# DavidBluecame/libYafaRay

Hardware: AMD Instinct MI355X
Metric: Mrays/sec + Msamples/sec, 1920×1080×64spp path-trace at 1/2/4/8 GPUs (higher is better)
Workload: dtype f32

## Files before the change

libyafaray_amd/csrc/kernels.hip:

```cpp

#include <hip/hip_runtime.h>
#include <cstdlib>
#include <string>
#include "devmath.h"
#include "photonheap.h"
#include "devscene.h"
#include "texeval.h"

namespace yafamd
{

#ifndef YAF_TRACE_BLOCK
#define YAF_TRACE_BLOCK 128
#endif
#ifndef YAF_SHADE_MIN_WAVES
#define YAF_SHADE_MIN_WAVES 4
#endif
#ifndef YAF_SHADE_LEAN_WAVES
#define YAF_SHADE_LEAN_WAVES 4
#endif
#ifndef YAF_SHADE_PREFETCH
#define YAF_SHADE_PREFETCH 1
#endif
constexpr int kTraceBlock = YAF_TRACE_BLOCK;
#ifdef YAF_EXPERIMENTS
constexpr bool kExperiments = true;
#else
constexpr bool kExperiments = false;
#endif
#if defined(YAF_FUSE) && defined(YAF_EXPERIMENTS)
constexpr bool kShadeFused = true;
#else
constexpr bool kShadeFused = false;
#endif
#ifndef YAF_FUSE_LEAN
#define YAF_FUSE_LEAN 0
#endif
constexpr int kShadeBlock = 256;

enum : uint32_t
{
	ST_CAMERA = 0,
	ST_FIRST = 1,
	ST_BOUNCE = 2,
	ST_NORAY = 3
};
enum : uint32_t
{
	F_MATFLAGS = 0xffffu,
	F_SAMPLED = 1u << 16,
	F_CAUSTIC = 1u << 17,
	F_PEND_V0 = 1u << 18,
	F_PEND_ONE = 1u << 19,
// ... 159 lines not shown
	Q.ray_d[3 * (size_t)i] = __builtin_nanf("");
}

constexpr uint32_t kPmSBits = 20, kPmLBits = 11;
__device__ __forceinline__ bool neePm8(const DevScene &S)
{
	return !S.nee_pm16 && (uint32_t)S.spp < (1u << kPmSBits) && S.n_lights <= (1 << kPmLBits);
}
typedef uint32_t u32x2_t __attribute__((ext_vector_type(2)));
#ifdef YAF_CHECKED
__device__ uint32_t g_nee_pm_err = 0;
#define NEE_PM_GUARD(cond) do { if(!(cond)) atomicCAS(&g_nee_pm_err, 0u, (uint32_t)__LINE__); } while(0)
#else
#define NEE_PM_GUARD(cond) do {} while(0)
#endif
__device__ __forceinline__ void neePmStore(const DevScene &S, uint4 *pm, uint32_t j, uint32_t offset, uint32_t sample_idx, uint32_t mode_l)
{
	if(neePm8(S))
	{
		NEE_PM_GUARD(sample_idx - S.base_offset - S.pass_offset < (uint32_t)S.spp);
		u32x2_t w;
		w.x = offset;
		w.y = (sample_idx - S.base_offset - S.pass_offset) | ((mode_l & 1u) << kPmSBits) | ((mode_l >> 8) << (kPmSBits + 1));
#if YAF_NT_STORE2
		__builtin_nontemporal_store(w, reinterpret_cast<u32x2_t *>(pm) + j);
#else
		reinterpret_cast<u32x2_t *>(pm)[j] = w;
#endif
	}
	else stStore2(&pm[j], make_uint4(offset, sample_idx, mode_l, 0u));
// ... 159 lines not shown
	{
		const uint32_t hstart = S.base_offset + S.pass_offset + offset;
		const float lu = haltonNext(3u, hstart, sc.s + 1), lv = haltonNext(5u, hstart, sc.s + 1);
		float u, v;
		lensUv(c, lu, lv, u, v);
		const V3 li = v3(c.dof_rt[0], c.dof_rt[1], c.dof_rt[2]) * u + v3(c.dof_up[0], c.dof_up[1], c.dof_up[2]) * v;
		from = from + li;
		dir = normalize(dir * c.dof_distance - li);
	}
	const uint64_t gid = ((uint64_t)sc.y * (uint64_t)S.width + (uint64_t)sc.x) * (uint64_t)S.spp + (uint64_t)sc.s;
	const uint32_t gid32 = (uint32_t)gid ^ fnv32((uint32_t)(gid >> 32));
	seed = fnv32(gid32 ^ S.rr_seed ^ (S.pass_offset * 0x9e3779b9u)) + 123u;
}

__global__ void __launch_bounds__(256) k_camera(DevScene S, DevPaths P, DevQueues Q, DevCounters cnt,
                                                 const DevJob *jobs, int n_jobs, uint64_t chunk_base, int n)
{
	const int i = blockIdx.x * blockDim.x + threadIdx.x;
	if((uint32_t)i < S.n_seg)
	{
		const uint32_t groups = (uint32_t)n / 256u, rem = (uint32_t)n % 256u, sg = (uint32_t)i, R = S.n_seg;
		cnt.n_active[sg] = (groups / R) * 256u + (sg < groups % R ? 256u : 0u) + (sg == groups % R ? rem : 0u);
		cnt.n_shadow[sg] = 0;
	}
	if(i >= n) return;
	const uint32_t g = (uint32_t)i / 256u;
	const uint32_t a = (g % S.n_seg) * S.cap_a + (g / S.n_seg) * 256u + (uint32_t)i % 256u;
	const SampleCoord sc = sampleAt(S, jobs, n_jobs, chunk_base + (uint64_t)i);
	V3 from, dir;
	float tmin, tmax;
	uint32_t seed;
	cameraRay(S, sc, from, dir, tmin, tmax, seed);
	storeQRay(Q, a, from, dir);
	if(S.cam.ray_tt) Q.ray_tt[a] = make_float2(tmin, tmax);
	if(!S.tree) reinterpret_cast<uint2 *>(P.pr)[a] = make_uint2((uint32_t)i, ST_CAMERA);
	else
	{
		const int cx = sc.x + S.crop_x0, cy = sc.y + S.crop_y0;
		const uint32_t offset = fnv32((uint32_t)cy * fnv32((uint32_t)cx));
		const uint32_t sample_idx = S.base_offset + S.pass_offset + (uint32_t)sc.s;
		Q.slot[a] = i;
		P.thr[a] = make_float4(0.f, 0.f, 0.f, 0.f);
		P.col[a] = make_float4(0.f, 0.f, 0.f, __uint_as_float(ST_CAMERA));
		P.pcol[a] = make_float4(0.f, 0.f, 0.f, __uint_as_float(0u));
		P.pr[a] = make_uint4(offset, sample_idx, 30903u, seed);
	}
}

#ifndef YAF_TOP_STRIDE
#define YAF_TOP_STRIDE 9
// ... 1978 lines not shown
struct ShadeArgs
{
	DevScene S;
	DevPaths Pc;
	DevPaths Pn;
	DevQueues Q;
	DevQueues Qn;
	DevNeeQueue N;
	DevNeeQueue G;
	DevCounters cnt;
	DevCounters cnt_next;
	float4 *samples;
	const DevJob *jobs;
	int n_jobs;
	uint64_t chunk_base;
};

__device__ __forceinline__ void writeSampleAt(const ShadeArgs &A, const SampleCoord &sc, C3 col, float alpha)
{
	if(alpha > 1.f) alpha = 1.f;
	A.samples[((size_t)sc.y * A.S.width + sc.x) * A.S.spp + sc.s] = f4(col, alpha);
}

__device__ __forceinline__ void writeSample(const ShadeArgs &A, uint32_t sid, C3 col, float alpha)
{
	writeSampleAt(A, sampleAt(A.S, A.jobs, A.n_jobs, A.chunk_base + (uint64_t)sid), col, alpha);
}

__device__ __forceinline__ Surf surfFromPrim(const DevScene &S, V3 p, int prim)
{
	Surf s;
// ... 33 lines not shown
				float f = m.tbias;
				if(m.sd_flags & SD_TBIAS_MULT) f *= (float)level;
				from = sp.p + dir * f;
			}
			S.spawn_o[idx] = f4(from, S.ray_min_dist);
			S.spawn_d[idx] = f4(dir, -1.f - (float)additional_depth);
			S.spawn_pr[idx] = make_uint4(pix.x, pix.y, rng.x ^ (0x9e3779b9u * (uint32_t)(2 * level + k + 1)), rng.y + 1u + (uint32_t)k);
			S.node_w[S.node_base + idx] = f4(k == 0 ? so.rcol : so.tcol, 0.f);
			if(k == 0) child.x = (int)(S.node_base + idx);
			else child.y = (int)(S.node_base + idx);
		}
	}
	S.node_child[node] = child;
}

template<bool SMALL, bool EXT, bool FUSED = false, bool LEAN = false, bool DEFER = false>
__global__ void __launch_bounds__(kShadeBlock, EXT ? 1 : (LEAN ? YAF_SHADE_LEAN_WAVES : YAF_SHADE_MIN_WAVES)) k_shade(ShadeArgs A)
{
	extern __shared__ uint4 shade_smem[];
	DevScene S_ = stageTables<SMALL>(A.S, shade_smem);
	if constexpr(LEAN)
	{
		S_.integrator = INT_PATH;
		S_.path_samples = 1;
		S_.do_ao = 0;
		S_.caus_map = 0;
		S_.show_map = 0;
		S_.gather_on = 0;
		S_.n_photons = 0;
		S_.fg_on = 0;
		S_.tree = 0;
		S_.has_attr = 0;
	}
// ... 11 lines not shown
	out.sh_count = &s_count[2];
	out.sh_base = seg * S.cap_s;
	out.Qn = A.Qn;
	out.idx_in_o = !S.tr_shad;
	const bool is_path = S.integrator == INT_PATH;
	const bool is_photon = S.integrator == INT_PHOTON;
	const bool keep_v0 = S.path_samples > 1 || is_photon || S.caus_map;
	const bool ao_after_caustic = S.caus_map && S.integrator == INT_DIRECT;
	const uint32_t n_paths = (uint32_t)max(1, S.path_samples);
	const int K = S.nee_k;
	const uint32_t stride = blockDim.x;
	const bool compact = !(EXT && S.tree);
	PHASE_DECL
#if YAF_SHADE_PREFETCH
	uint2 pr_n = make_uint2(0u, ST_NORAY);
	if(compact && threadIdx.x < n_a) pr_n = reinterpret_cast<const uint2 *>(Pc.pr)[a0 + threadIdx.x];
#endif
	for(uint32_t base_j = 0; base_j < n_a; base_j += stride)
	{
		const bool live = base_j + threadIdx.x < n_a;
		const uint32_t i = a0 + base_j + threadIdx.x;
#if YAF_SHADE_PREFETCH
		const uint2 pr_cur = pr_n;
		if(compact && base_j + stride + threadIdx.x < n_a) pr_n = reinterpret_cast<const uint2 *>(Pc.pr)[i + stride];
#endif
		uint32_t sid = 0, stage = ST_NORAY, flags = 0;
		uint2 pix = make_uint2(0u, 0u), rng = make_uint2(0u, 0u);
		float w = 0.f;
		float4 thr4 = make_float4(0.f, 0.f, 0.f, 0.f), col4 = thr4, pcol4 = thr4, pwo4 = thr4, pthr4 = thr4, pem4 = thr4;
		float4 v0p4 = thr4, v0wo4 = thr4;
		float4 v0a0 = thr4, v0a1 = thr4;
		SampleCoord sc{0, 0, 0};
		if(live)
		{
			if(compact)
			{
#if YAF_SHADE_PREFETCH
				const uint2 pr = pr_cur;
#else
				const uint2 pr = reinterpret_cast<const uint2 *>(Pc.pr)[i];
#endif
				sid = pr.x;
				stage = pr.y;
				sc = sampleAt(S, A.jobs, A.n_jobs, A.chunk_base + (uint64_t)sid);
				pix = make_uint2(fnv32((uint32_t)(sc.y + S.crop_y0) * fnv32((uint32_t)(sc.x + S.crop_x0))),
				                 S.base_offset + S.pass_offset + (uint32_t)sc.s);
			}
			else
			{
				const uint4 pr = Pc.pr[i];
				rng = make_uint2(pr.z, pr.w);
				sid = (uint32_t)A.Q.slot[i];
				pix = make_uint2(pr.x, pr.y);
				col4 = Pc.col[i];
				stage = __float_as_uint(col4.w);
			}
			if(!compact || (stage & 0xffu) != ST_CAMERA)
			{
				if(S.w_live) thr4 = Pc.thr[i];
				else
				{
					const F3 t = reinterpret_cast<const F3 *>(Pc.thr)[i];
					thr4 = make_float4(t.x, t.y, t.z, 0.f);
				}
				pcol4 = Pc.pcol[i];
				if(keep_v0) { v0p4 = Pc.v0p[i]; v0wo4 = Pc.v0wo[i]; }
				if(ATTR && keep_v0) { v0a0 = Pc.v0attr[2 * (size_t)i]; v0a1 = Pc.v0attr[2 * (size_t)i + 1]; }
			}
			w = thr4.w;
			flags = __float_as_uint(pcol4.w);
			if((stage & 0xffu) == ST_FIRST && !(flags & F_SAMPLED)) pwo4 = Pc.pwo[i];
			if(flags & F_PEND_ONE)
			{
				const F3 t = reinterpret_cast<const F3 *>(Pc.pend_thr)[i];
				pthr4 = make_float4(t.x, t.y, t.z, 0.f);
			}
			if(flags & (F_PEND_EMIT | F_AO_EMIT)) pem4 = Pc.pend_emit[i];
		}
		C3 thr = rgb(thr4), col = rgb(col4), pcol = rgb(pcol4);
		const float alpha = 1.f;
		V3 pwo = xyz(pwo4);
		const uint32_t st = stage & 0xffu;
		uint32_t subpath = (stage >> 8) & 0xfffu;
		int depth = (int)(stage >> 20);
		const uint32_t offset = pix.x, sample_idx = pix.y;
		C3 ao_extra = c3(0.f);
		bool col_ld = !compact, col_dirty = false;
		auto loadCol = [&]() {
			if(!col_ld)
			{
				col = (flags & F_COLS) ? rgb(Pc.csmp[sid]) : c3(0.f);
				col_ld = true;
			}
		};

		PHASE(0);
		const int kb = (int)i * K;
// ... 241 lines not shown
					if(S.caustic_path && (s.sampled & (B_SPECULAR | B_GLOSSY | B_FILTER))) flags |= F_CAUSTIC;
					else flags &= ~F_CAUSTIC;
					ray_o = sp.p;
					ray_d = dir;
					want_ray = true;
					stage = ST_BOUNCE | (subpath << 8) | ((uint32_t)depth << 20);
				}
			}
			else end_sub = true;
		}
		if(live && end_sub && !pending)
		{
			if(is_path && (flags & F_V0_DIFFUSE) && subpath + 1 < n_paths) { start_sub = true; ++subpath; }
			else finalize = true;
		}
		if(live && start_sub)
		{
			Surf s0 = (st == ST_CAMERA) ? sp : surfFromPrim(S, xyz(v0p4), __float_as_int(v0p4.w));
			if(ATTR && st != ST_CAMERA) applyAttr(s0, v0a0, v0a1);
			const V3 wo0 = (st == ST_CAMERA) ? wo : xyz(v0wo4);
			const uint32_t offs = n_paths * sample_idx + offset + subpath;
			BsdfSample s;
			s.s_1 = riVdC(offs);
			s.s_2 = ldsDim(S, 2, offs);
			s.flags = B_DIFFUSE | B_REFLECT | B_TRANSMIT;
			s.pdf = 0.f;
			s.sampled = B_NONE;
			V3 dir = v3(0.f, 0.f, 0.f);
			C3 scol = matSample<EXT>(S.mats[s0.mat], s0, wo0, dir, s, w);
			thr = scol * w;
// ... 55 lines not shown
			else
			{
				storeQNoRay(A.Qn, k);
				if(!FUSED && want_nee) reinterpret_cast<F3 *>(A.Qn.ray_o)[k] = F3{sp.p.x, sp.p.y, sp.p.z};
				stage = ST_NORAY | (subpath << 8) | ((uint32_t)depth << 20);
			}
			if(compact) stStoreU2(reinterpret_cast<uint2 *>(Pn.pr) + k, make_uint2(sid, stage));
			else
			{
				stStore(&Pn.pr[k], make_uint4(pix.x, pix.y, rng.x, rng.y));
				stStore(&Pn.col[k], f4(col, __uint_as_float(stage)));
			}
			if(S.w_live) stStore(&Pn.thr[k], f4(thr, w));
			else stStoreF3(Pn.thr, k, thr);
			stStore(&Pn.pcol[k], f4(pcol, __uint_as_float(flags)));
			if((stage & 0xffu) == ST_FIRST && !(flags & F_SAMPLED)) Pn.pwo[k] = f4(pwo, 0.f);
			if(nee_one) reinterpret_cast<F3 *>(Pn.pend_thr)[k] = F3{pend_thr.r, pend_thr.g, pend_thr.b};
			if(flags & (F_PEND_EMIT | F_AO_EMIT)) Pn.pend_emit[k] = f4(emit_pend, 0.f);
			if(keep_v0) { Pn.v0p[k] = v0p4; Pn.v0wo[k] = v0wo4; }
			if(ATTR && keep_v0) { Pn.v0attr[2 * (size_t)k] = v0a0; Pn.v0attr[2 * (size_t)k + 1] = v0a1; }
		}

		PHASE(4);
		if(FUSED)
		{
			const int e0 = (int)k * K;
			const bool all = live && nee_v0, one = live && nee_one;
			const DevMaterial &m = S.mats[sp.mat];
			float4 *ts = S.tr_shad ? Pn.ts : nullptr;
			if(__any(all))
			{
// ... 3285 lines not shown
using namespace yafamd;

extern "C" {

int yafamd_trace_block() { return kTraceBlock; }

int yafamd_shade_fused() { return kShadeFused ? 1 : 0; }
int yafamd_shade_fused_for(const DevScene *S)
{
	if(S->ext) return 0;
	if(kShadeFused) return 1;
	return (YAF_FUSE_LEAN && S->integrator == INT_PATH && S->path_samples <= 1 && !S->do_ao && !S->caus_map && !S->gather_on && !S->show_map &&
	        S->n_photons == 0 && !S->tree && !S->has_attr && !S->no_lean && !S->tr_shad && !S->has_mesh_light) ? 1 : 0;
}

int yafamd_experiments() { return kExperiments ? 1 : 0; }

#ifndef YAF_DEVICE_BUILD
#define YAF_DEVICE_BUILD "arch=? extra=[?] (built outside csrc/Makefile)"
#endif
const char *yafamd_device_build() { return YAF_DEVICE_BUILD
#ifdef YAF_PHASE_TIMING
	" phase-timing"
#endif
	; }

int yafamd_phase_cycles(unsigned long long *out, int n, int reset)
{
#ifdef YAF_PHASE_TIMING
	unsigned long long h[16];
// ... 37 lines not shown
int yafamd_nee_blocks_per_cu()
{
	int nb = 0;
	if(hipOccupancyMaxActiveBlocksPerMultiprocessor(&nb, (k_nee<true, false>), kShadeBlock, 8192) != hipSuccess) nb = 0;
	return nb;
}

int yafamd_shade_blocks_per_cu()
{
	int nb = 0;
	if(hipOccupancyMaxActiveBlocksPerMultiprocessor(&nb, (k_shade<true, false>), kShadeBlock, 8192) != hipSuccess) nb = 0;
	return nb;
}

hipError_t yafamd_launch_camera(const DevScene *S, const DevPaths *P, const DevQueues *Q, const DevCounters *cnt,
                                const DevJob *jobs, int n_jobs, uint64_t chunk_base, int n, hipStream_t st)
{
	if(n <= 0) return hipSuccess;
	const int threads = max(n, (int)S->n_seg);
	hipLaunchKernelGGL(k_camera, dim3((threads + 255) / 256), dim3(256), 0, st, *S, *P, *Q, *cnt, jobs, n_jobs, chunk_base, n);
	return hipGetLastError();
}

hipError_t yafamd_launch_trace(const DevScene *S, const DevQueues *Q, const DevCounters *cnt, const DevPaths *P,
                               DevStats *stats, int stack_depth, int *spill, int grid, hipStream_t st)
{
	const size_t stack_bytes = (size_t)stack_depth * kTraceBlock * sizeof(int);
	const bool wide = S->node_f4 == 8;
	const size_t lds_scene = S->scene_in_lds ? (size_t)(S->node_f4 * S->n_nodes + 3 * S->n_tris) * sizeof(float4)
	                                         : (wide ? (size_t)S->lds_top * kTopStride * sizeof(float4) : 0);
	const size_t bytes = stack_bytes + lds_scene;
	if(S->nodes8 && !S->scene_in_lds && !S->tr_shad)
	{
		const size_t bytes8 = stack_bytes + (size_t)S->lds_top8 * kTop8Stride * sizeof(float4);
		if(S->trace_stats)
// ... 56 lines not shown
			                   stack_depth, spill);
	}
#endif
	else if(wide && !S->trace_stats)
		hipLaunchKernelGGL((k_trace<false, true, false, true, false>), dim3(grid), dim3(kTraceBlock), bytes, st, *S, *Q, *cnt, *P, stats,
		                   stack_depth, spill);
	else if(wide) YAF_TRACE_LAUNCH(false, true, false, true);
	else YAF_TRACE_LAUNCH(false, false, false, true);
#undef YAF_TRACE_LAUNCH
	return hipGetLastError();
}

hipError_t yafamd_launch_shade(const DevScene *S, const DevPaths *Pc, const DevPaths *Pn, const DevQueues *Q,
                               const DevQueues *Qn, const DevNeeQueue *N, const DevNeeQueue *G, const DevCounters *cnt,
                               const DevCounters *cnt_next, float4 *samples, const DevJob *jobs, int n_jobs, uint64_t chunk_base,
                               hipStream_t st)
{
	ShadeArgs A;
	A.S = *S;
	A.Pc = *Pc;
	A.Pn = *Pn;
	A.Q = *Q;
	A.Qn = *Qn;
	A.N = *N;
	A.G = *G;
	A.cnt = *cnt;
	A.cnt_next = *cnt_next;
	A.samples = samples;
	A.jobs = jobs;
	A.n_jobs = n_jobs;
	A.chunk_base = chunk_base;
	const size_t lds = shadeLdsBytes(*S, S->small_tables != 0);
	if(S->lpc_mode == 3)
// ... 7 lines not shown
		else hipLaunchKernelGGL((k_shade<false, false, false, false, true>), dim3(S->n_seg), dim3(kShadeBlock), lds, st, A);
		return hipGetLastError();
	}
	if(S->ext)
	{
		if(S->small_tables) hipLaunchKernelGGL((k_shade<true, true>), dim3(S->n_seg), dim3(kShadeBlock), lds, st, A);
		else hipLaunchKernelGGL((k_shade<false, true>), dim3(S->n_seg), dim3(kShadeBlock), lds, st, A);
	}
	else if(!kShadeFused && S->integrator == INT_PATH && S->path_samples <= 1 && !S->do_ao && !S->caus_map && !S->gather_on && !S->show_map &&
	        S->n_photons == 0 && !S->tree && !S->has_attr && !S->no_lean)
	{
		if(yafamd_shade_fused_for(S))
		{
			if(S->small_tables) hipLaunchKernelGGL((k_shade<true, false, true, true>), dim3(S->n_seg), dim3(kShadeBlock), lds, st, A);
			else hipLaunchKernelGGL((k_shade<false, false, true, true>), dim3(S->n_seg), dim3(kShadeBlock), lds, st, A);
		}
		else if(S->small_tables) hipLaunchKernelGGL((k_shade<true, false, false, true>), dim3(S->n_seg), dim3(kShadeBlock), lds, st, A);
		else hipLaunchKernelGGL((k_shade<false, false, false, true>), dim3(S->n_seg), dim3(kShadeBlock), lds, st, A);
	}
	else if(S->small_tables) hipLaunchKernelGGL((k_shade<true, false, kShadeFused>), dim3(S->n_seg), dim3(kShadeBlock), lds, st, A);
	else hipLaunchKernelGGL((k_shade<false, false, kShadeFused>), dim3(S->n_seg), dim3(kShadeBlock), lds, st, A);
	return hipGetLastError();
}

int yafamd_dfr_eligible(const DevScene *S)
{
	if(S->n_lights > kDfrMaxLights) return 0;
	if(S->integrator != INT_PATH || S->ext || S->tree || S->gather_on || S->tr_shad || S->has_attr || S->caus_map || S->do_ao) return 0;
	const char *e = getenv("YAFARAY_AMD_LIGHT_PICK");
	return (e && std::string(e) == "count") ? 0 : 1;
// ... 500 lines not shown
```

libyafaray_amd/csrc/render.cc:

```cpp
#include "render.h"
#include "devmath.h"
#include "photonfile.h"

#include <hip/hip_runtime.h>
#include <rccl/rccl.h>

#include <algorithm>
#include <array>
#include <chrono>
#include <cmath>
#include <cstdlib>
#include <cstring>
#include <future>
#include <mutex>
#include <sstream>
#include <unordered_map>

using namespace yafamd;

extern "C" {
hipError_t yafamd_launch_camera(const DevScene *S, const DevPaths *P, const DevQueues *Q, const DevCounters *cnt,
                                const DevJob *jobs, int n_jobs, uint64_t chunk_base, int n, hipStream_t st);
hipError_t yafamd_launch_surface(const DevScene *S, const DevQueues *Q, const DevCounters *cnt, hipStream_t st);
hipError_t yafamd_launch_tshadow(const DevScene *S, const DevQueues *Q, const DevCounters *cnt, const DevPaths *P, hipStream_t st);
hipError_t yafamd_launch_spawn(const DevScene *S, const DevPaths *P, const DevQueues *Q, const DevCounters *cnt, uint32_t s0, int n,
                               hipStream_t st);
hipError_t yafamd_launch_combine(const DevScene *S, uint32_t lo, uint32_t hi, int final_level, float4 *samples, const DevJob *jobs,
                                 int n_jobs, uint64_t chunk_base, hipStream_t st);
hipError_t yafamd_launch_trace(const DevScene *S, const DevQueues *Q, const DevCounters *cnt, const DevPaths *P,
                               DevStats *stats, int stack_depth, int *spill, int grid, hipStream_t st);
int yafamd_trace_block();
int yafamd_shade_fused();
int yafamd_walk_lds_levels(int pm_stack);
int yafamd_walk_threads(const DevScene *S);
int yafamd_shade_fused_for(const DevScene *S);
int yafamd_experiments();
int yafamd_trace_blocks_per_cu(int lds_scene, int wide, size_t dyn_lds);
int yafamd_shade_blocks_per_cu();
hipError_t yafamd_launch_shade(const DevScene *S, const DevPaths *Pc, const DevPaths *Pn, const DevQueues *Q,
                               const DevQueues *Qn, const DevNeeQueue *N, const DevNeeQueue *G, const DevCounters *cnt,
                               const DevCounters *cnt_next, float4 *samples, const DevJob *jobs, int n_jobs, uint64_t chunk_base,
                               hipStream_t st);
int yafamd_path_eligible(const DevScene *S, int stack_depth, int spill);
int yafamd_path_blocks_per_cu(const DevScene *S, int stack_depth);
hipError_t yafamd_launch_path(const DevScene *S, float4 *samples, const DevJob *jobs, int n_jobs, uint64_t chunk_base, uint32_t n,
                              uint32_t *next, int stack_depth, int grid, hipStream_t st);
hipError_t yafamd_launch_nee(const DevScene *S, const DevNeeQueue *N, const DevPaths *Pn, const DevQueues *Qn,
                             const DevCounters *cnt_next, int stack_depth, hipStream_t st);
int yafamd_nee_blocks_per_cu();
hipError_t yafamd_photon_emit(const DevScene *S, const PhotonState *P, const PhotonSet *L, uint32_t n_photons, uint32_t h0, uint32_t n_local,
                              int max_bounces, hipStream_t st);
hipError_t yafamd_photon_bounce(const DevScene *S, const PhotonState *P, const PhotonSet *L, uint32_t n_photons, uint32_t h0,
                                uint32_t n_local, int max_bounces, int bounce, int cur, int stack_depth, int *spill, int grid, hipStream_t st);
hipError_t yafamd_photon_compact(const PhotonState *P, uint32_t *scratch_counts, uint32_t *total_dev, float4 *pos, float4 *dir, float *colb,
                                 hipStream_t st);
hipError_t yafamd_launch_gather(const DevScene *S, const DevNeeQueue *G, const DevCounters *cnt_next, float4 *samples,
                                const DevJob *jobs, int n_jobs, uint64_t chunk_base, const GatherLogDesc *log, hipStream_t st);
// ... 2037 lines not shown
	if(const char *e = std::getenv("YAFARAY_AMD_OVERLAP_SHADOW_GRID"); e && atoi(e) > 0)
		ov_shadow_grid = (int)S.n_seg * std::max(1, std::min(atoi(e), d.trace_grid) / (int)S.n_seg);
	ov_shadow = ov_shadow && overlap && d.spill.p == nullptr;
	bool lpc_on = S.integrator == INT_PATH && S.n_lights > 1 && !S.tree && (rp.shard_world <= 1 || group_render);
	if(const char *lp = std::getenv("YAFARAY_AMD_LIGHT_PICK"); lp && std::string(lp) == "hash") lpc_on = false;
	lpc_carry_ = 0;
	S.lpc = nullptr;
	S.lpc_mode = 0;
	S.nee_pm16 = 0;
	if(const char *e = std::getenv("YAFARAY_AMD_NEE_PM16"); e && *e == '1') S.nee_pm16 = 1;
	if(const char *e = std::getenv("YAFARAY_AMD_W_LIVE"); e && *e == '1') S.w_live = 1;
	S.no_lean = 0;
	S.fg_probe = 0;
	if(const char *e = std::getenv("YAFARAY_AMD_FG_PROBE"); e && *e) S.fg_probe = atoi(e);
	if(const char *e = std::getenv("YAFARAY_AMD_SHADE_LEAN"); e && *e == '0') S.no_lean = 1;
	int path_grid = 0;
	if(!lpc_on)
	{
		const char *pe = std::getenv("YAFARAY_AMD_PATH");
		const bool on = yafamd_experiments() && pe && std::string(pe) == "mega";
		if(on && yafamd_path_eligible(&S, d.lds_stack, d.lds_stack < d.stack_depth ? 1 : 0))
		{
			path_grid = std::min(d.trace_grid, d.n_cu * std::max(1, yafamd_path_blocks_per_cu(&S, d.lds_stack)));
			if(const char *e = getenv("YAFARAY_AMD_PATH_GRID")) path_grid = std::min(d.trace_grid, std::max(1, atoi(e)));
			if(!ensure(log_, d.path_next, 16)) return false;
		}
	}
	const int n_paths = std::max(1, S.path_samples);
	const int iters = (S.integrator == INT_PATH) ? 2 + n_paths * (S.bounces + 2) : 3;

	auto ensureEvents = [&](size_t need) -> bool {
		while(d.ev_pool.size() < need)
		{
			hipEvent_t e;
			HIPCHECK(hipEventCreate(&e));
			d.ev_pool.push_back(e);
		}
		return true;
	};
	if(!ensureEvents(2)) return false;
	HIPCHECK(hipEventRecord(d.ev_pool[0], d.stream));
	DevStats *run_stats = dstats;
	auto iterate = [&](uint64_t base) -> bool {
		int cur = 0;
		const bool count_run = S.lpc_mode == 1;
		bool closest_done = false;
		for(int it = 0; it < iters; ++it)
		{
			DevQueues qc = d.Q[cur];
			if(it != 0 || (S.cur_level == 0 && !S.cam.ray_tt)) qc.ray_tt = nullptr;
			qc.tmin_dflt = it == 0 ? 0.f : S.ray_min_dist;
			qc.perm = nullptr;
			qc.trace_part = closest_done ? TRACE_SHADOW : TRACE_BOTH;
			const bool join_pending = closest_done && ov_shadow;
			closest_done = false;
			if(ray_bin && it >= 1 && !count_run)
			{
				size_t tb = d.bin_tmp.bytes;
// ... 11 lines not shown
				}();
				if(!ok)
				{
					(void)hipStreamSynchronize(d.side);
					return false;
				}
			}
			else
				PROF(KK_TRACE, yafamd_launch_trace(&S, &qc, &cnt[cur], &d.P[cur], run_stats, d.lds_stack, (int *)d.spill.p,
				                                    S.tr_shad ? d.trace_grid_bvh4 : d.trace_grid, d.stream));
			if(S.tr_shad && !count_run) PROF(KK_TSHADOW, yafamd_launch_tshadow(&S, &qc, &cnt[cur], &d.P[cur], d.stream));
			if(S.has_attr) PROF(KK_SURFACE, yafamd_launch_surface(&S, &qc, &cnt[cur], d.stream));
			if(S.lpc_mode == 3)
				HIPCHECK(yafamd_dfr_segoff(&cnt[cur], S.n_seg, (uint32_t *)d.dfr_segoff.p, (uint32_t *)d.dfr_misc.p, S.dfr_cap,
				                           (uint32_t *)d.dfr_misc.p + 1, (uint32_t *)d.dfr_its.p, d.stream));
			PROF(KK_SHADE, yafamd_launch_shade(&S, &d.P[cur], &d.P[cur ^ 1], &qc, &d.Q[cur ^ 1], &d.N, &d.G, &cnt[cur], &cnt[cur ^ 1],
			                             (float4 *)d.samples.p, (const DevJob *)d.jobs.p, n_jobs, base, d.stream));

			const bool dl_pipeline = S.integrator != INT_PATH;
			if(S.gather_on && !count_run && (!dl_pipeline || it == 1 || (S.show_map && it == 0)))
			{
				if(S.fg_on && fg_paths)
				{
					if(!fgPrepare()) return false;
					for(uint32_t j0 = 0; j0 < S.cap_a; j0 += fgb.seg_cap)
					{
						FgBatch B = fgb;
						B.j0 = j0;
						HIPCHECK(hipMemsetAsync(fgb.long_count, 0, (size_t)S.n_seg * 4, d.stream));
						PROF(KK_FG, yafamd_launch_fg_paths(&S, &d.G, &cnt[cur ^ 1], d.lds_stack, (int *)d.spill.p, d.trace_grid, &B, d.stream));
					}
				}
// ... 58 lines not shown
		if(rp.on_chunk && base > 0)
		{
			HIPCHECK(hipStreamSynchronize(d.stream));
			rp.on_chunk(base, n_total);
			if(canceled && *canceled) break;
		}
		if(path_grid > 0)
		{
			HIPCHECK(hipMemsetAsync(d.path_next.p, 0, 4, d.stream));
			PROF(KK_PATH, yafamd_launch_path(&S, (float4 *)d.samples.p, (const DevJob *)d.jobs.p, n_jobs, base, (uint32_t)n, (uint32_t *)d.path_next.p,
			                                 d.lds_stack, path_grid, d.stream));
			continue;
		}
		if(S.tree) HIPCHECK(hipMemsetAsync(d.spawn_count.p, 0, 16, d.stream));
		S.cur_level = 0;
		PROF(KK_CAMERA, yafamd_launch_camera(&S, &d.P[0], &d.Q[0], &cnt[0], (const DevJob *)d.jobs.p, n_jobs, base, n, d.stream));
		if(!iterate(base)) return false;
		if(!S.tree) continue;
		std::vector<std::pair<uint32_t, uint32_t>> levels;
		uint32_t done = 0;
		for(int level = 1;; ++level)
		{
			uint32_t hc[2] = {0, 0};
			HIPCHECK(hipMemcpyAsync(hc, d.spawn_count.p, 8, hipMemcpyDeviceToHost, d.stream));
			HIPCHECK(hipStreamSynchronize(d.stream));
			if(hc[1] && !tree_overflow_logged)
			{
				log_.error("Integrator: the specular recursion tree exceeded its " + std::to_string(S.spawn_cap) + " node records; deeper rays dropped");
				tree_overflow_logged = true;
			}
			const uint32_t total_spawned = std::min(hc[0], S.spawn_cap);
// ... 376 lines not shown
		S.pass_offset = 0;
		S.plist = nullptr;
		S.fg_pass_samples = 0;
		rp.film.spp = spp;
		if(light_mult)
		{
			HIPCHECK(hipStreamSynchronize(d.stream));
			lightLayout(1.f, d.pass_lights);
			HIPCHECK(hipMemcpy(d.lights.p, d.pass_lights.data(), d.pass_lights.size() * sizeof(DevLight), hipMemcpyHostToDevice));
		}
	}
	HIPCHECK(hipEventRecord(d.ev_pool[1], d.stream));
	HIPCHECK(hipStreamSynchronize(d.stream));
	float ms = 0.f;
	HIPCHECK(hipEventElapsedTime(&ms, d.ev_pool[0], d.ev_pool[1]));
	DevStats hs{};
	{
		std::vector<DevStats> per_block(2 * (size_t)d.trace_grid);
		HIPCHECK(hipMemcpy(per_block.data(), d.stats.p, sizeof(DevStats) * per_block.size(), hipMemcpyDeviceToHost));
		for(const DevStats &b : per_block)
		{
			hs.closest_rays += b.closest_rays;
			hs.shadow_rays += b.shadow_rays;
			hs.node_visits += b.node_visits;
			hs.tri_tests += b.tri_tests;
			hs.shade_entries += b.shade_entries;
			hs.nee_requests += b.nee_requests;
			hs.gather_queries += b.gather_queries;
			hs.gather_visits += b.gather_visits;
			hs.gather_photons += b.gather_photons;
// ... 480 lines not shown
```

libyafaray_amd/csrc/render.h:

```cpp
#pragma once

#include "bvh.h"
#include "devscene.h"
#include "host.h"

#include <condition_variable>
#include <cstdint>
#include <functional>
#include <memory>
#include <mutex>
#include <string>
#include <vector>

namespace yafamd
{


struct HostScene
{
	BvhOutput bvh;
	bool gpu_build = false;
	std::vector<float> verts;
	std::vector<int> tris;
	int ploc_iters = 0;
// ... 45 lines not shown
{
	int passes = 1;
	int inc_samples = 1;
	float light_sample_multiplier_factor = 1.f;
	float indirect_sample_multiplier_factor = 1.f;
	float threshold = 0.05f;
	float resampled_floor = 0.f;
	float sample_multiplier_factor = 1.f;
	DevAaParams dev{0, 0, 0.f, 10, 0};
};

enum KernelKind : int
{
	KK_CAMERA = 0, KK_TRACE, KK_SURFACE, KK_TSHADOW, KK_SHADE, KK_NEE, KK_GATHER, KK_SPAWN, KK_COMBINE, KK_FILM, KK_AA,
	KK_PHOTON_EMIT, KK_PHOTON_BOUNCE, KK_PHOTON_COMPACT, KK_PHOTON_TREE, KK_FG, KK_PREGATHER, KK_GATHER_WALK, KK_PATH, KK_DFR,
	KK_LAYER_HITS, KK_LAYER_FILM, KK_COUNT
};
inline const char *kernelKindName(int k)
{
	static const char *n[KK_COUNT] = {"k_camera", "k_trace", "k_surface", "k_tshadow", "k_shade", "k_nee", "k_gather", "k_spawn",
	                                  "k_combine", "k_film", "aa_next_pass", "k_photon_emit", "k_photon_bounce", "photon_compact",
	                                  "pkd_build", "k_fg", "k_pregather", "k_gather_walk", "k_path", "k_dfr", "k_layer_hits", "k_layer_film"};
	return (k >= 0 && k < KK_COUNT) ? n[k] : "";
}
struct KernelTimes
{
	double ms[KK_COUNT] = {};
	uint64_t launches[KK_COUNT] = {};
	uint64_t items[KK_COUNT] = {};
};

struct LayerParams
{
	std::vector<int> kinds;
	std::vector<float> mat_index;
	std::vector<int> obj_seg;
	float mat_highest = 1.f, obj_highest = 1.f;
// ... 132 lines not shown
```

Measured before the change: 2248.

## Specialise lean shade kernel per wavefront stage and skip camera pr writes

Adds stage-specialised instantiations of the lean k_shade kernel (camera, first-hit, bounce). In these the stage is known at compile time, so stage-dependent branches, pwo loads and stores, and pending-flag handling fold away. For the camera stage the path record is recomputed from the thread index instead of being read, and k_camera no longer writes it. A device error counter checks the stage assumptions and the host fails the render if any are violated, which adds atomics on the guard path, an extra host readback, and more kernel variants to compile.

```diff
diff --git a/libyafaray_amd/csrc/kernels.hip b/libyafaray_amd/csrc/kernels.hip
--- a/libyafaray_amd/csrc/kernels.hip
+++ b/libyafaray_amd/csrc/kernels.hip
@@ -37,6 +37,12 @@
 #define YAF_FUSE_LEAN 0
 #endif
 constexpr int kShadeBlock = 256;
+#ifndef YAF_SHADE_CAMERA_BLOCK
+#define YAF_SHADE_CAMERA_BLOCK 256
+#endif
+constexpr int kShadeCameraBlock = YAF_SHADE_CAMERA_BLOCK;
+
+enum : int { SG_ANY = 0, SG_CAMERA = 1, SG_FIRST = 2, SG_BOUNCE = 3 };
 
 enum : uint32_t
 {
@@ -226,6 +232,8 @@
 #else
 #define NEE_PM_GUARD(cond) do {} while(0)
 #endif
+constexpr int kStageErrWords = 32;
+__device__ uint32_t g_shade_stage_err[kStageErrWords] = {};
 __device__ __forceinline__ void neePmStore(const DevScene &S, uint4 *pm, uint32_t j, uint32_t offset, uint32_t sample_idx, uint32_t mode_l)
 {
 	if(neePm8(S))
@@ -415,7 +423,7 @@
 }
 
 __global__ void __launch_bounds__(256) k_camera(DevScene S, DevPaths P, DevQueues Q, DevCounters cnt,
-                                                 const DevJob *jobs, int n_jobs, uint64_t chunk_base, int n)
+                                                 const DevJob *jobs, int n_jobs, uint64_t chunk_base, int n, int write_pr)
 {
 	const int i = blockIdx.x * blockDim.x + threadIdx.x;
 	if((uint32_t)i < S.n_seg)
@@ -434,7 +442,10 @@
 	cameraRay(S, sc, from, dir, tmin, tmax, seed);
 	storeQRay(Q, a, from, dir);
 	if(S.cam.ray_tt) Q.ray_tt[a] = make_float2(tmin, tmax);
-	if(!S.tree) reinterpret_cast<uint2 *>(P.pr)[a] = make_uint2((uint32_t)i, ST_CAMERA);
+	if(!S.tree)
+	{
+		if(write_pr) reinterpret_cast<uint2 *>(P.pr)[a] = make_uint2((uint32_t)i, ST_CAMERA);
+	}
 	else
 	{
 		const int cx = sc.x + S.crop_x0, cy = sc.y + S.crop_y0;
@@ -2443,7 +2454,17 @@
 	const DevJob *jobs;
 	int n_jobs;
 	uint64_t chunk_base;
+	int stage_it;
 };
+
+template<int STAGE>
+__device__ __forceinline__ uint32_t stageOf(uint32_t stage)
+{
+	if constexpr(STAGE == SG_CAMERA) return ST_CAMERA;
+	else if constexpr(STAGE == SG_FIRST) return ST_FIRST;
+	else if constexpr(STAGE == SG_BOUNCE) return (stage & 0xffu) == ST_NORAY ? ST_NORAY : ST_BOUNCE;
+	else return stage & 0xffu;
+}
 
 __device__ __forceinline__ void writeSampleAt(const ShadeArgs &A, const SampleCoord &sc, C3 col, float alpha)
 {
@@ -2507,9 +2528,12 @@
 	S.node_child[node] = child;
 }
 
-template<bool SMALL, bool EXT, bool FUSED = false, bool LEAN = false, bool DEFER = false>
-__global__ void __launch_bounds__(kShadeBlock, EXT ? 1 : (LEAN ? YAF_SHADE_LEAN_WAVES : YAF_SHADE_MIN_WAVES)) k_shade(ShadeArgs A)
-{
+template<bool SMALL, bool EXT, bool FUSED = false, bool LEAN = false, bool DEFER = false, int STAGE = SG_ANY>
+__global__ void __launch_bounds__(STAGE == SG_CAMERA ? kShadeCameraBlock : kShadeBlock,
+                                  STAGE == SG_CAMERA ? kShadeCameraBlock / 64 : (EXT ? 1 : (LEAN ? YAF_SHADE_LEAN_WAVES : YAF_SHADE_MIN_WAVES)))
+k_shade(ShadeArgs A)
+{
+	static_assert(STAGE == SG_ANY || (LEAN && !EXT && !FUSED && !DEFER), "a fixed stage is the lean non-fused kernel's");
 	extern __shared__ uint4 shade_smem[];
 	DevScene S_ = stageTables<SMALL>(A.S, shade_smem);
 	if constexpr(LEAN)
@@ -2551,7 +2575,7 @@
 	PHASE_DECL
 #if YAF_SHADE_PREFETCH
 	uint2 pr_n = make_uint2(0u, ST_NORAY);
-	if(compact && threadIdx.x < n_a) pr_n = reinterpret_cast<const uint2 *>(Pc.pr)[a0 + threadIdx.x];
+	if(STAGE != SG_CAMERA && compact && threadIdx.x < n_a) pr_n = reinterpret_cast<const uint2 *>(Pc.pr)[a0 + threadIdx.x];
 #endif
 	for(uint32_t base_j = 0; base_j < n_a; base_j += stride)
 	{
@@ -2559,7 +2583,7 @@
 		const uint32_t i = a0 + base_j + threadIdx.x;
 #if YAF_SHADE_PREFETCH
 		const uint2 pr_cur = pr_n;
-		if(compact && base_j + stride + threadIdx.x < n_a) pr_n = reinterpret_cast<const uint2 *>(Pc.pr)[i + stride];
+		if(STAGE != SG_CAMERA && compact && base_j + stride + threadIdx.x < n_a) pr_n = reinterpret_cast<const uint2 *>(Pc.pr)[i + stride];
 #endif
 		uint32_t sid = 0, stage = ST_NORAY, flags = 0;
 		uint2 pix = make_uint2(0u, 0u), rng = make_uint2(0u, 0u);
@@ -2573,12 +2597,20 @@
 			if(compact)
 			{
 #if YAF_SHADE_PREFETCH
-				const uint2 pr = pr_cur;
+				uint2 pr = pr_cur;
 #else
-				const uint2 pr = reinterpret_cast<const uint2 *>(Pc.pr)[i];
-#endif
+				uint2 pr = make_uint2(0u, ST_CAMERA);
+				if(STAGE != SG_CAMERA) pr = reinterpret_cast<const uint2 *>(Pc.pr)[i];
+#endif
+				if constexpr(STAGE == SG_CAMERA)
+				{
+					const uint32_t off = i - a0;
+					pr = make_uint2(((off / 256u) * S.n_seg + seg) * 256u + off % 256u, ST_CAMERA);
+				}
 				sid = pr.x;
 				stage = pr.y;
+				if constexpr(STAGE == SG_FIRST || STAGE == SG_BOUNCE)
+					if(stageOf<STAGE>(stage) != (stage & 0xffu)) atomicAdd(&g_shade_stage_err[min(A.stage_it, kStageErrWords - 1)], 1u);
 				sc = sampleAt(S, A.jobs, A.n_jobs, A.chunk_base + (uint64_t)sid);
 				pix = make_uint2(fnv32((uint32_t)(sc.y + S.crop_y0) * fnv32((uint32_t)(sc.x + S.crop_x0))),
 				                 S.base_offset + S.pass_offset + (uint32_t)sc.s);
@@ -2592,7 +2624,7 @@
 				col4 = Pc.col[i];
 				stage = __float_as_uint(col4.w);
 			}
-			if(!compact || (stage & 0xffu) != ST_CAMERA)
+			if(!compact || stageOf<STAGE>(stage) != ST_CAMERA)
 			{
 				if(S.w_live) thr4 = Pc.thr[i];
 				else
@@ -2606,7 +2638,17 @@
 			}
 			w = thr4.w;
 			flags = __float_as_uint(pcol4.w);
-			if((stage & 0xffu) == ST_FIRST && !(flags & F_SAMPLED)) pwo4 = Pc.pwo[i];
+			if constexpr(STAGE == SG_FIRST)
+			{
+				if(flags & F_PEND_ONE) atomicAdd(&g_shade_stage_err[min(A.stage_it, kStageErrWords - 1)], 1u);
+				flags &= ~F_PEND_ONE;
+			}
+			if constexpr(STAGE == SG_BOUNCE)
+			{
+				if(flags & F_PEND_V0) atomicAdd(&g_shade_stage_err[min(A.stage_it, kStageErrWords - 1)], 1u);
+				flags &= ~F_PEND_V0;
+			}
+			if(stageOf<STAGE>(stage) == ST_FIRST && !(flags & F_SAMPLED)) pwo4 = Pc.pwo[i];
 			if(flags & F_PEND_ONE)
 			{
 				const F3 t = reinterpret_cast<const F3 *>(Pc.pend_thr)[i];
@@ -2617,7 +2659,7 @@
 		C3 thr = rgb(thr4), col = rgb(col4), pcol = rgb(pcol4);
 		const float alpha = 1.f;
 		V3 pwo = xyz(pwo4);
-		const uint32_t st = stage & 0xffu;
+		const uint32_t st = stageOf<STAGE>(stage);
 		uint32_t subpath = (stage >> 8) & 0xfffu;
 		int depth = (int)(stage >> 20);
 		const uint32_t offset = pix.x, sample_idx = pix.y;
@@ -2889,6 +2931,7 @@
 			if(is_path && (flags & F_V0_DIFFUSE) && subpath + 1 < n_paths) { start_sub = true; ++subpath; }
 			else finalize = true;
 		}
+		if constexpr(STAGE == SG_FIRST || STAGE == SG_BOUNCE) start_sub = false;
 		if(live && start_sub)
 		{
 			Surf s0 = (st == ST_CAMERA) ? sp : surfFromPrim(S, xyz(v0p4), __float_as_int(v0p4.w));
@@ -2974,7 +3017,7 @@
 			if(S.w_live) stStore(&Pn.thr[k], f4(thr, w));
 			else stStoreF3(Pn.thr, k, thr);
 			stStore(&Pn.pcol[k], f4(pcol, __uint_as_float(flags)));
-			if((stage & 0xffu) == ST_FIRST && !(flags & F_SAMPLED)) Pn.pwo[k] = f4(pwo, 0.f);
+			if((STAGE == SG_ANY || STAGE == SG_CAMERA) && (stage & 0xffu) == ST_FIRST && !(flags & F_SAMPLED)) Pn.pwo[k] = f4(pwo, 0.f);
 			if(nee_one) reinterpret_cast<F3 *>(Pn.pend_thr)[k] = F3{pend_thr.r, pend_thr.g, pend_thr.b};
 			if(flags & (F_PEND_EMIT | F_AO_EMIT)) Pn.pend_emit[k] = f4(emit_pend, 0.f);
 			if(keep_v0) { Pn.v0p[k] = v0p4; Pn.v0wo[k] = v0wo4; }
@@ -6290,6 +6333,30 @@
 	        S->n_photons == 0 && !S->tree && !S->has_attr && !S->no_lean && !S->tr_shad && !S->has_mesh_light) ? 1 : 0;
 }
 
+int yafamd_shade_stages_for(const DevScene *S)
+{
+	return (!S->ext && !kShadeFused && S->integrator == INT_PATH && S->path_samples <= 1 && !S->do_ao && !S->caus_map && !S->gather_on && !S->show_map &&
+	        S->n_photons == 0 && !S->tree && !S->has_attr && !S->no_lean && !yafamd_shade_fused_for(S)) ? 1 : 0;
+}
+
+int yafamd_shade_stage_errors(uint32_t *out, int n)
+{
+	uint32_t h[kStageErrWords];
+	if(hipMemcpyFromSymbol(h, HIP_SYMBOL(g_shade_stage_err), sizeof(h)) != hipSuccess) return 0;
+	bool any = false;
+	for(int k = 0; k < kStageErrWords; ++k)
+	{
+		if(k < n) out[k] = h[k];
+		any = any || h[k] != 0u;
+	}
+	if(any)
+	{
+		const uint32_t z[kStageErrWords] = {};
+		if(hipMemcpyToSymbol(HIP_SYMBOL(g_shade_stage_err), z, sizeof(z)) != hipSuccess) return 0;
+	}
+	return kStageErrWords;
+}
+
 int yafamd_experiments() { return kExperiments ? 1 : 0; }
 
 #ifndef YAF_DEVICE_BUILD
@@ -6357,11 +6424,11 @@
 }
 
 hipError_t yafamd_launch_camera(const DevScene *S, const DevPaths *P, const DevQueues *Q, const DevCounters *cnt,
-                                const DevJob *jobs, int n_jobs, uint64_t chunk_base, int n, hipStream_t st)
+                                const DevJob *jobs, int n_jobs, uint64_t chunk_base, int n, int write_pr, hipStream_t st)
 {
 	if(n <= 0) return hipSuccess;
 	const int threads = max(n, (int)S->n_seg);
-	hipLaunchKernelGGL(k_camera, dim3((threads + 255) / 256), dim3(256), 0, st, *S, *P, *Q, *cnt, jobs, n_jobs, chunk_base, n);
+	hipLaunchKernelGGL(k_camera, dim3((threads + 255) / 256), dim3(256), 0, st, *S, *P, *Q, *cnt, jobs, n_jobs, chunk_base, n, write_pr);
 	return hipGetLastError();
 }
 
@@ -6448,9 +6515,11 @@
 hipError_t yafamd_launch_shade(const DevScene *S, const DevPaths *Pc, const DevPaths *Pn, const DevQueues *Q,
                                const DevQueues *Qn, const DevNeeQueue *N, const DevNeeQueue *G, const DevCounters *cnt,
                                const DevCounters *cnt_next, float4 *samples, const DevJob *jobs, int n_jobs, uint64_t chunk_base,
-                               hipStream_t st)
-{
+                               int stage_it, hipStream_t st)
+{
+	if(stage_it >= 0 && !(yafamd_shade_stages_for(S) && S->cur_level == 0 && S->lpc_mode == 0)) return hipErrorInvalidValue;
 	ShadeArgs A;
+	A.stage_it = max(stage_it, 0);
 	A.S = *S;
 	A.Pc = *Pc;
 	A.Pn = *Pn;
@@ -6488,6 +6557,18 @@
 		{
 			if(S->small_tables) hipLaunchKernelGGL((k_shade<true, false, true, true>), dim3(S->n_seg), dim3(kShadeBlock), lds, st, A);
 			else hipLaunchKernelGGL((k_shade<false, false, true, true>), dim3(S->n_seg), dim3(kShadeBlock), lds, st, A);
+		}
+		else if(stage_it >= 0)
+		{
+#define YAF_SHADE_STAGE_LAUNCH(SM) \
+			do { \
+				if(stage_it == 0) hipLaunchKernelGGL((k_shade<SM, false, false, true, false, SG_CAMERA>), dim3(S->n_seg), dim3(kShadeCameraBlock), lds, st, A); \
+				else if(stage_it == 1) hipLaunchKernelGGL((k_shade<SM, false, false, true, false, SG_FIRST>), dim3(S->n_seg), dim3(kShadeBlock), lds, st, A); \
+				else hipLaunchKernelGGL((k_shade<SM, false, false, true, false, SG_BOUNCE>), dim3(S->n_seg), dim3(kShadeBlock), lds, st, A); \
+			} while(0)
+			if(S->small_tables) YAF_SHADE_STAGE_LAUNCH(true);
+			else YAF_SHADE_STAGE_LAUNCH(false);
+#undef YAF_SHADE_STAGE_LAUNCH
 		}
 		else if(S->small_tables) hipLaunchKernelGGL((k_shade<true, false, false, true>), dim3(S->n_seg), dim3(kShadeBlock), lds, st, A);
 		else hipLaunchKernelGGL((k_shade<false, false, false, true>), dim3(S->n_seg), dim3(kShadeBlock), lds, st, A);
diff --git a/libyafaray_amd/csrc/render.cc b/libyafaray_amd/csrc/render.cc
--- a/libyafaray_amd/csrc/render.cc
+++ b/libyafaray_amd/csrc/render.cc
@@ -20,7 +20,7 @@
 
 extern "C" {
 hipError_t yafamd_launch_camera(const DevScene *S, const DevPaths *P, const DevQueues *Q, const DevCounters *cnt,
-                                const DevJob *jobs, int n_jobs, uint64_t chunk_base, int n, hipStream_t st);
+                                const DevJob *jobs, int n_jobs, uint64_t chunk_base, int n, int write_pr, hipStream_t st);
 hipError_t yafamd_launch_surface(const DevScene *S, const DevQueues *Q, const DevCounters *cnt, hipStream_t st);
 hipError_t yafamd_launch_tshadow(const DevScene *S, const DevQueues *Q, const DevCounters *cnt, const DevPaths *P, hipStream_t st);
 hipError_t yafamd_launch_spawn(const DevScene *S, const DevPaths *P, const DevQueues *Q, const DevCounters *cnt, uint32_t s0, int n,
@@ -40,7 +40,9 @@
 hipError_t yafamd_launch_shade(const DevScene *S, const DevPaths *Pc, const DevPaths *Pn, const DevQueues *Q,
                                const DevQueues *Qn, const DevNeeQueue *N, const DevNeeQueue *G, const DevCounters *cnt,
                                const DevCounters *cnt_next, float4 *samples, const DevJob *jobs, int n_jobs, uint64_t chunk_base,
-                               hipStream_t st);
+                               int stage_it, hipStream_t st);
+int yafamd_shade_stages_for(const DevScene *S);
+int yafamd_shade_stage_errors(uint32_t *out, int n);
 int yafamd_path_eligible(const DevScene *S, int stack_depth, int spill);
 int yafamd_path_blocks_per_cu(const DevScene *S, int stack_depth);
 hipError_t yafamd_launch_path(const DevScene *S, float4 *samples, const DevJob *jobs, int n_jobs, uint64_t chunk_base, uint32_t n,
@@ -2108,6 +2110,8 @@
 	S.fg_probe = 0;
 	if(const char *e = std::getenv("YAFARAY_AMD_FG_PROBE"); e && *e) S.fg_probe = atoi(e);
 	if(const char *e = std::getenv("YAFARAY_AMD_SHADE_LEAN"); e && *e == '0') S.no_lean = 1;
+	bool shade_stages = !lpc_on && yafamd_shade_stages_for(&S) != 0;
+	if(const char *e = std::getenv("YAFARAY_AMD_SHADE_STAGES"); e && *e == '0') shade_stages = false;
 	int path_grid = 0;
 	if(!lpc_on)
 	{
@@ -2135,7 +2139,8 @@
 	if(!ensureEvents(2)) return false;
 	HIPCHECK(hipEventRecord(d.ev_pool[0], d.stream));
 	DevStats *run_stats = dstats;
-	auto iterate = [&](uint64_t base) -> bool {
+	bool shade_staged = false;
+	auto iterate =[&](uint64_t base) -> bool {
 		int cur = 0;
 		const bool count_run = S.lpc_mode == 1;
 		bool closest_done = false;
@@ -2177,8 +2182,14 @@
 			if(S.lpc_mode == 3)
 				HIPCHECK(yafamd_dfr_segoff(&cnt[cur], S.n_seg, (uint32_t *)d.dfr_segoff.p, (uint32_t *)d.dfr_misc.p, S.dfr_cap,
 				                           (uint32_t *)d.dfr_misc.p + 1, (uint32_t *)d.dfr_its.p, d.stream));
+			const int stage_it = (shade_stages && S.cur_level == 0 && S.lpc_mode == 0 && !S.tree) ? it : -1;
 			PROF(KK_SHADE, yafamd_launch_shade(&S, &d.P[cur], &d.P[cur ^ 1], &qc, &d.Q[cur ^ 1], &d.N, &d.G, &cnt[cur], &cnt[cur ^ 1],
-			                             (float4 *)d.samples.p, (const DevJob *)d.jobs.p, n_jobs, base, d.stream));
+			                             (float4 *)d.samples.p, (const DevJob *)d.jobs.p, n_jobs, base, stage_it, d.stream));
+			if(stage_it >= 0)
+			{
+				shade_staged = true;
+				if(rp.profile) ++ktimes_.launches[KK_SHADE_STAGED];
+			}
 
 			const bool dl_pipeline = S.integrator != INT_PATH;
 			if(S.gather_on && !count_run && (!dl_pipeline || it == 1 || (S.show_map && it == 0)))
@@ -2267,7 +2278,7 @@
 		}
 		if(S.tree) HIPCHECK(hipMemsetAsync(d.spawn_count.p, 0, 16, d.stream));
 		S.cur_level = 0;
-		PROF(KK_CAMERA, yafamd_launch_camera(&S, &d.P[0], &d.Q[0], &cnt[0], (const DevJob *)d.jobs.p, n_jobs, base, n, d.stream));
+		PROF(KK_CAMERA, yafamd_launch_camera(&S, &d.P[0], &d.Q[0], &cnt[0], (const DevJob *)d.jobs.p, n_jobs, base, n, shade_stages ? 0 : 1, d.stream));
 		if(!iterate(base)) return false;
 		if(!S.tree) continue;
 		std::vector<std::pair<uint32_t, uint32_t>> levels;
@@ -2674,6 +2685,23 @@
 	HIPCHECK(hipStreamSynchronize(d.stream));
 	float ms = 0.f;
 	HIPCHECK(hipEventElapsedTime(&ms, d.ev_pool[0], d.ev_pool[1]));
+	if(shade_staged)
+	{
+		uint32_t err[32] = {};
+		const int n_err = yafamd_shade_stage_errors(err, 32);
+		if(n_err <= 0)
+		{
+			log_.error("Integrator: the stage guard of k_shade could not be read");
+			return false;
+		}
+		for(int k = 0; k < n_err && k < 32; ++k)
+			if(err[k])
+			{
+				log_.error("Integrator: k_shade iteration " + std::to_string(k) + (k == n_err - 1 ? " or later" : "") + " met " + std::to_string(err[k]) +
+				           " entries of another stage than its stage-specialised kernel handles (YAFARAY_AMD_SHADE_STAGES=0 renders without them)");
+				return false;
+			}
+	}
 	DevStats hs{};
 	{
 		std::vector<DevStats> per_block(2 * (size_t)d.trace_grid);
diff --git a/libyafaray_amd/csrc/render.h b/libyafaray_amd/csrc/render.h
--- a/libyafaray_amd/csrc/render.h
+++ b/libyafaray_amd/csrc/render.h
@@ -83,13 +83,16 @@
 {
 	KK_CAMERA = 0, KK_TRACE, KK_SURFACE, KK_TSHADOW, KK_SHADE, KK_NEE, KK_GATHER, KK_SPAWN, KK_COMBINE, KK_FILM, KK_AA,
 	KK_PHOTON_EMIT, KK_PHOTON_BOUNCE, KK_PHOTON_COMPACT, KK_PHOTON_TREE, KK_FG, KK_PREGATHER, KK_GATHER_WALK, KK_PATH, KK_DFR,
-	KK_LAYER_HITS, KK_LAYER_FILM, KK_COUNT
+	KK_LAYER_HITS, KK_LAYER_FILM,
+	KK_SHADE_STAGED,
+	KK_COUNT
 };
 inline const char *kernelKindName(int k)
 {
 	static const char *n[KK_COUNT] = {"k_camera", "k_trace", "k_surface", "k_tshadow", "k_shade", "k_nee", "k_gather", "k_spawn",
 	                                  "k_combine", "k_film", "aa_next_pass", "k_photon_emit", "k_photon_bounce", "photon_compact",
-	                                  "pkd_build", "k_fg", "k_pregather", "k_gather_walk", "k_path", "k_dfr", "k_layer_hits", "k_layer_film"};
+	                                  "pkd_build", "k_fg", "k_pregather", "k_gather_walk", "k_path", "k_dfr", "k_layer_hits", "k_layer_film",
+	                                  "k_shade_staged"};
 	return (k >= 0 && k < KK_COUNT) ? n[k] : "";
 }
 struct KernelTimes
```

Result: faster. 2292 (median of 6 runs) (+2.0%).
